# bdsaglam/torch-scae

Hardware: AMD Instinct MI355X
Metric: images/sec SCAE fwd+bwd, MNIST 40x40 bs=128, 1/2/4/8 MI355X (higher is better)
Workload: dtype f32

## Files before the change

### torch_scae_amd/csrc/seed_attention_wave.hip

```cpp
#include <algorithm>

#include "wave_mfma.h"

using namespace scae_wave;

namespace {
constexpr int NTH = 256;

struct SwArgs {
  const float *h;
  const float *q;
  const float *wk;
  const float *wv, *bv;
  const float *presence;
  float *out;
  const float *gout;
  float *gh;
  float *partial;
  int B, N, O, C;
  float inv_sqrt_c;
  int bf16;
};

enum { T_QK = 0, T_TS, T_DT, T_QKT, T_TT, T_DTT, T_SMALL };
// ... 162 lines not shown
  fold_qk<NT>(a, l, tl, false);
  for (int b = blockIdx.x; b < a.B; b += gridDim.x) {
    if (l.v < NT && 16 * l.v < O) {
      const int t = l.v;
      const Keys<NT> k = load_keys<NT>(a, b, l);
      f32x4 p[NT];
      probabilities<NT, BF>(a, l, tl, t, k, p);
      wr_nn<NT>(tl.large(T_PS), t, l, p);
      lds_fence();
      const f32x4 T = mmakp<NT, BF>(splat(0.f), rdk<NT>(tl.large(T_PS), t, l), k.hT);
      wr_rows(tl.small(T_TS), t, l, T);
      lds_fence();
    }
    __syncthreads();
    float *ob = a.out + (size_t)b * O * C;
    for (int ct = l.v; ct * 16 < C; ct += 4) {
      const float4 wb = ld4(a.wv + (size_t)(16 * ct + l.r) * D + 4 * l.q);
      const float bias = a.bv[16 * ct + l.r];
#pragma unroll
      for (int t = 0; t < NT; ++t) {
        if (16 * t >= O) break;
        const f32x4 o = mma16(splat(bias), rd16(tl.small(T_TS), t, l), wb);
#pragma unroll
        for (int e = 0; e < 4; ++e) {
          const int row = 16 * t + 4 * l.q + e;
          if (row < O) ob[(size_t)row * C + 16 * ct + l.r] = o[e];
        }
      }
    }
    __syncthreads();
  }
}

template <int NT, bool BF>
__device__ __forceinline__ f32x4 saw_bwd_body(const SwArgs &a, float *smem, int blk, int nblk) {
  const Tl<NT> tl{smem};
  const Lane l = make_lane();
  const int C = a.C, O = a.O, N = a.N, CW = C / 4, run = CW / 4;
  constexpr int TSN = Geo<NT>::TSN;
  const int npar = O * D + C * D + C;
  float *part = a.partial + (size_t)blk * npar;
  float *scr = tl.scr();
  static_assert(Geo<NT>::LDS_FLOATS % 4 == 0, "16-byte zero fill");
  for (int i = 4 * threadIdx.x; i < Geo<NT>::LDS_FLOATS; i += 4 * NTH)
    *reinterpret_cast<float4 *>(smem + i) = make_float4(0.f, 0.f, 0.f, 0.f);
  __syncthreads();
  fold_qk<NT>(a, l, tl, true);
  bool first = true;
  auto put = [&](int idx, float v) { part[idx] = first ? v : part[idx] + v; };
  const int k0 = CW * l.v + run * l.q;
  f32x4 gh_tile = splat(0.f);
  for (int b = blk; b < a.B; b += nblk) {
    const float *gb = a.gout + (size_t)b * O * C;
    {
      f32x4 acc[NT];
#pragma unroll
      for (int t = 0; t < NT; ++t) acc[t] = splat(0.f);
      for (int j = 0; j < run; j += 4) {
        const float *wp = a.wv + (size_t)(k0 + j) * D + l.r;
        const float4 wb = make_float4(wp[0], wp[D], wp[2 * D], wp[3 * D]);
#pragma unroll
        for (int t = 0; t < NT; ++t) {
          const int o = 16 * t + l.r;
          const float4 av =
              o < O ? ld4(gb + (size_t)o * C + k0 + j) : make_float4(0.f, 0.f, 0.f, 0.f);
          acc[t] = mma16(acc[t], av, wb);
        }
      }
#pragma unroll
      for (int t = 0; t < NT; ++t)
#pragma unroll
        for (int e = 0; e < 4; ++e)
          scr[((l.v * NT + t) * 16 + 4 * l.q + e) * D + l.r] = acc[t][e];
    }
    Keys<NT> k;
    f32x4 p[NT];
    const bool qwave = l.v < NT && 16 * l.v < O;
    if (qwave) {
      const int t = l.v;
      k = load_keys<NT>(a, b, l);
      probabilities<NT, BF>(a, l, tl, t, k, p);
      wr_nn<NT>(tl.large(T_PS), t, l, p);
      wr_nn_t<NT>(tl.large(T_PT), t, l, p);
      lds_fence();
      const f32x4 T = mmakp<NT, BF>(splat(0.f), rdk<NT>(tl.large(T_PS), t, l), k.hT);
      wr_cols<NT>(tl.small(T_TT), t, l, T);
    }
    lds_fence();
    __syncthreads();
    for (int i = threadIdx.x; i < Geo<NT>::ROWS * D; i += NTH) {
      const float s =
          (scr[i] + scr[NT * 256 + i]) + (scr[2 * NT * 256 + i] + scr[3 * NT * 256 + i]);
      const int o = i / D, c = i % D;
      tl.small(T_DT)[o * RS + c] = s;
      tl.small(T_DTT)[c * TSN + o] = s;
    }
    __syncthreads();
    {
      const FK<NT> tb = rdk<NT>(tl.small(T_TT), 0, l);
      for (int ct = l.v; ct * 16 < C; ct += 4) {
        FK<NT> ga;
        float cs = 0.f;
#pragma unroll
        for (int j = 0; j < NT; ++j) {
          float g[4];
#pragma unroll
          for (int s = 0; s < 4; ++s) {
            const int o = 4 * NT * l.q + 4 * j + s;
            g[s] = o < O ? gb[(size_t)o * C + 16 * ct + l.r] : 0.f;
          }
          ga.v[j] = make_float4(g[0], g[1], g[2], g[3]);
          cs += (g[0] + g[1]) + (g[2] + g[3]);
        }
        const f32x4 dw = mmak<NT>(splat(0.f), ga, tb);
#pragma unroll
        for (int e = 0; e < 4; ++e) put(O * D + (16 * ct + 4 * l.q + e) * D + l.r, dw[e]);
        cs += __shfl_xor(cs, 16, 64);
        cs += __shfl_xor(cs, 32, 64);
        if (l.q == 0) put(O * D + C * D + 16 * ct + l.r, cs);
      }
    }
    if (qwave) {
      const int t = l.v;
      const float4 dta = rd16(tl.small(T_DT), t, l);
      f32x4 ds[NT];
#pragma unroll
      for (int u = 0; u < NT; ++u) ds[u] = mma16p<BF>(splat(0.f), dta, k.hB[u]);
#pragma unroll
      for (int e = 0; e < 4; ++e) {
        float dot = 0.f;
#pragma unroll
        for (int u = 0; u < NT; ++u) dot = fmaf(p[u][e], ds[u][e], dot);
        dot = rsum(dot);
#pragma unroll
        for (int u = 0; u < NT; ++u) ds[u][e] = p[u][e] * (ds[u][e] - dot) * a.inv_sqrt_c;
      }
      wr_nn<NT>(tl.large(T_DSR), t, l, ds);
      wr_nn_t<NT>(tl.large(T_DST), t, l, ds);
      lds_fence();
      const f32x4 dqk = mmakp<NT, BF>(splat(0.f), rdk<NT>(tl.large(T_DSR), t, l), k.hT);
#pragma unroll
      for (int e = 0; e < 4; ++e) {
        const int o = 16 * t + 4 * l.q + e;
        if (o < O) put(o * D + l.r, dqk[e]);
      }
    }
    lds_fence();
    __syncthreads();
    if (l.v < NT && 16 * l.v < N) {
      const int u = l.v;
      f32x4 gh = mmakp<NT, BF>(splat(0.f), rdk<NT>(tl.large(T_PT), u, l), rdk<NT>(tl.small(T_DTT), 0, l));
      gh = mmakp<NT, BF>(gh, rdk<NT>(tl.large(T_DST), u, l), rdk<NT>(tl.small(T_QKT), 0, l));
#pragma unroll
      for (int e = 0; e < 4; ++e) {
        const int n = 16 * u + 4 * l.q + e;
        if (n < N) a.gh[((size_t)b * N + n) * D + l.r] = gh[e];
      }
      gh_tile = gh;
    }
    first = false;
    __syncthreads();
  }
  return gh_tile;
}
template <int NT, bool BF>
__global__ __launch_bounds__(NTH) void saw_bwd_kernel(SwArgs a) {
  extern __shared__ __attribute__((aligned(16))) float smem[];
  saw_bwd_body<NT, BF>(a, smem, blockIdx.x, gridDim.x);
}

constexpr int RTH = 1024;
struct ReduceArgs {
  const float *partial;
  int rows;
  const float *q, *wk;
  float *gq, *gwk, *gbk, *gwv, *gbv;
  int O, C, nsum;
};
inline int reduce_blocks(const ReduceArgs &r, int RT) {
  return r.nsum + (r.O * r.C + r.C * D + RT - 1) / RT;
}
template <int RT>
__device__ __forceinline__ void saw_reduce_body(const ReduceArgs &a, float *lds, int blk) {
  constexpr int VR = RTH / RT;
  float (*red)[65] = reinterpret_cast<float (*)[65]>(lds);
  float *dqk = lds + 16 * 65;
  const float *__restrict__ partial = a.partial;
  const int rows = a.rows, O = a.O, C = a.C, nsum = a.nsum;
  const int npar = O * D + C * D + C;
  const int cx = threadIdx.x & 63, ry0 = (threadIdx.x >> 6) * VR;
  auto colsum = [&](int col, bool ok) {
#pragma unroll
    for (int vr = 0; vr < VR; ++vr) {
      const int ry = ry0 + vr;
      float acc = 0.f;
      if (ok) {
// ... 143 lines not shown
```

### torch_scae_amd/csrc/seed_bwd_gemm.hip

```cpp
#include <algorithm>

#include "mfma_tile.h"
#include "set_encoder_args.h"
#include "wave_mfma.h"

#define SCAE_DEVICE_ONLY
namespace scae_saw {
#include "seed_attention_wave.hip"
}
namespace scae_gemm {
#include "gemm_mfma.hip"
}
#include "set_encoder_wave.hip"
#undef SCAE_DEVICE_ONLY

namespace {
constexpr int NTH = 256;
static_assert(scae_tile::NT == NTH, "one block size for both parts");

template <int NT, bool BF>
__global__ __launch_bounds__(NTH) void saw_bwd_gemm_kernel(scae_saw::SwArgs a, int n_saw,
                                                           scae_gemm::GemmMulti p) {
  extern __shared__ __attribute__((aligned(16))) float smem[];
  if ((int)blockIdx.x < n_saw)
    scae_saw::saw_bwd_body<NT, BF>(a, smem, blockIdx.x, n_saw);
  else
    scae_gemm::gemm_multi_body<1>(p, smem, (int)blockIdx.x - n_saw);
}

template <int NT, bool BF>
int launch(const scae_saw::SwArgs &a, const scae_gemm::GemmMulti &p, hipStream_t st) {
  const size_t lds = sizeof(float) * std::max<size_t>(scae_saw::Geo<NT>::LDS_FLOATS,
                                                      scae_tile::Tile<1>::SMEM);
// ... 31 lines not shown
__global__ __launch_bounds__(NTH) __attribute__((amdgpu_waves_per_eu(2)))
void saw_stw_bwd_gemm_kernel(scae_saw::SwArgs a, int n_saw,
                                                               scae_gemm::GemmMulti p,
                                                               scae_st::StArgs t,
                                                               int trunk_lds_floats) {
  extern __shared__ __attribute__((aligned(16))) float smem[];
  if ((int)blockIdx.x >= n_saw) {
    scae_gemm::gemm_multi_body<1>(p, smem, (int)blockIdx.x - n_saw);
    return;
  }
  const scae_wave::f32x4 gh = scae_saw::saw_bwd_body<2, BF>(a, smem, blockIdx.x, n_saw);
  scae_st::lds_zero(smem, trunk_lds_floats, threadIdx.x, NTH);
  scae_wave::lds_fence();
  __syncthreads();
  if (threadIdx.x >= 64 * NTS) return;
  scae_st::stw_bwd_body<NTS, BF, true>(t, smem, blockIdx.x, n_saw, gh);
}

template <int NTS, bool BF>
int launch_trunk(const scae_saw::SwArgs &a, const scae_gemm::GemmMulti &p,
                 const scae_st::StArgs &t, hipStream_t st) {
  const size_t trunk = scae_st::stw_bwd_lds_floats<NTS>(t.Din);
  const size_t lds =
      sizeof(float) * std::max<size_t>({scae_saw::Geo<2>::LDS_FLOATS, scae_tile::Tile<1>::SMEM, trunk});
  if (lds > 48 * 1024) {
    hipError_t e = hipFuncSetAttribute(
        reinterpret_cast<const void *>(saw_stw_bwd_gemm_kernel<NTS, BF>),
        hipFuncAttributeMaxDynamicSharedMemorySize, (int)lds);
    if (e != hipSuccess) return (int)e;
  }
  scae::launch((saw_stw_bwd_gemm_kernel<NTS, BF>), dim3(a.B + p.first[p.n]), dim3(NTH), lds, st,
               a, a.B, p, t, (int)trunk);
  return scae_launch_status();
}

bool trunk_rides(int B, int N, int O, int C, int D, int Din, int Dout, int L, int layer_norm) {
  return B > 0 && B <= 512 && N > 0 && N <= 32 && O > 0 && O <= 32 && C > 0 && (C & 63) == 0 &&
         D == scae_wave::D && Dout == 0 && scae_st::wave_bwd_shape(N, D, Din, Dout, L, layer_norm);
}

int impl_trunk(const float *h, const float *q, const float *wk, const float *wv,
               const float *presence, const float *gout, float *gh, float *partial, int B, int N,
               int O, int C, const scae_gemm_desc *descs, int n, int nseg,
               const float *const *seg_ptr, const int *seg_width, const int *seg_row_stride,
               const int64_t *seg_batch_stride, float *const *seg_grad,
               const float *trunk_presence, const float *params, const float *hsave,
               float *pg_partial, int B2, int N2, int D, int Din, int Dout, int L, int layer_norm,
               int bf16, void *stream) {
  SCAE_REQUIRE(h && q && wk && wv && gout && gh && partial && descs);
  if (B2 != B || N2 != N) return SCAE_ERR_BAD_ARG;
  scae_saw::SwArgs a{h,  q,       wk, wv, nullptr, presence, nullptr, gout,
                     gh, partial, B,  N,  O,       C,        1.f / sqrtf((float)C), bf16};
  int rc = scae_saw::check(a);
  if (rc) return rc;
  scae_st::StArgs t;
  rc = scae_st::wave_bwd_args(t, bf16 != 0, nseg, seg_ptr, seg_width, seg_row_stride,
                              seg_batch_stride, seg_grad, trunk_presence, params, hsave,
                              pg_partial, B, N, D, Din, Dout, L, layer_norm);
  if (rc) return rc;
  scae_gemm::GemmMulti p;
  int T;
  rc = scae_gemm::plan_multi(p, T, descs, n);
  if (rc) return rc;
  if (T != 32) return SCAE_ERR_UNSUPPORTED;
  if (!trunk_rides(B, N, O, C, D, Din, Dout, L, layer_norm)) return SCAE_ERR_UNSUPPORTED;
  hipStream_t st = (hipStream_t)stream;
  if (N <= 16) return bf16 ? launch_trunk<1, true>(a, p, t, st) : launch_trunk<1, false>(a, p, t, st);
  return bf16 ? launch_trunk<2, true>(a, p, t, st) : launch_trunk<2, false>(a, p, t, st);
}
}

extern "C" int scae_object_encoder_bwd_supported(int B, int N, int O, int C, int D, int Din,
                                                 int Dout, int L, int layer_norm) {
  return trunk_rides(B, N, O, C, D, Din, Dout, L, layer_norm) ? 1 : 0;
}
#define SCAE_OBJECT_ENCODER_BWD(SUFFIX, BF)                                                      \
  extern "C" int scae_object_encoder_bwd_gemm_##SUFFIX(                                          \
      const float *h, const float *q, const float *wk, const float *wv, const float *presence,   \
      const float *gout, float *gh, float *partial, int B, int N, int O, int C,                  \
      const scae_gemm_desc *descs, int n, int nseg, const float *const *seg_ptr,                 \
      const int *seg_width, const int *seg_row_stride, const int64_t *seg_batch_stride,          \
      float *const *seg_grad, const float *trunk_presence, const float *params,                  \
      const float *hsave, float *pg_partial, int trunk_B, int trunk_N, int D, int Din, int Dout, \
      int L, int layer_norm, void *stream) {                                                     \
    return impl_trunk(h, q, wk, wv, presence, gout, gh, partial, B, N, O, C, descs, n, nseg,     \
                      seg_ptr, seg_width, seg_row_stride, seg_batch_stride, seg_grad,            \
                      trunk_presence, params, hsave, pg_partial, trunk_B, trunk_N, D, Din, Dout, \
                      L, layer_norm, BF, stream);                                                \
  }
SCAE_OBJECT_ENCODER_BWD(f32, 0)
SCAE_OBJECT_ENCODER_BWD(bf16, 1)
#undef SCAE_OBJECT_ENCODER_BWD

extern "C" int scae_seed_attention_mfma_bwd_gemm_f32(
    const float *h, const float *q, const float *wk, const float *wv, const float *presence,
    const float *gout, float *gh, float *partial, int B, int N, int O, int C,
    const scae_gemm_desc *descs, int n, void *stream) {
  return impl(h, q, wk, wv, presence, gout, gh, partial, B, N, O, C, descs, n, 0, stream);
}
extern "C" int scae_seed_attention_mfma_bwd_gemm_bf16(
    const float *h, const float *q, const float *wk, const float *wv, const float *presence,
    const float *gout, float *gh, float *partial, int B, int N, int O, int C,
    const scae_gemm_desc *descs, int n, void *stream) {
// ... 3 lines not shown
```

### torch_scae_amd/csrc/set_encoder_wave.hip

```cpp
#include "set_encoder_args.h"
#include "wave_mfma.h"

#pragma clang fp contract(off)

namespace scae_st {
namespace {
using namespace scae_wave;

#ifdef SCAE_STW_PROF
__device__ unsigned long long g_stw_prof[160];
__device__ int g_stw_n;
#define STW_T()                                                                  \
  do {                                                                           \
    if (blockIdx.x == 5 && threadIdx.x == 0) {                                   \
      const int i_ = g_stw_n;                                                    \
      if (i_ < 160) g_stw_prof[i_] = __builtin_readcyclecounter(), g_stw_n = i_ + 1; \
    }                                                                            \
  } while (0)
#else
#define STW_T()
#endif

struct Lay {
  int Din, L, ln;
  __device__ int b1() const { return D * Din; }
  __device__ int layer(int l) const { return D * Din + D + l * (5 * 272 + (ln ? 64 : 0)); }
  __device__ int w(int m) const { return m < 4 ? m * 272 : 4 * 272 + (ln ? 32 : 0); }
  __device__ int b(int m) const { return w(m) + 256; }
  __device__ int ln0() const { return 4 * 272; }
  __device__ int ln1() const { return b(4) + 16; }
  __device__ int total() const { return layer(L); }
};

struct Wave {
  int lane, r, q, t;
  int ts;
  __device__ __forceinline__ void wr_rows(float *tile, const f32x4 &o) const {
#pragma unroll
    for (int e = 0; e < 4; ++e) tile[(16 * t + 4 * q + e) * RS + r] = o[e];
  }
  __device__ __forceinline__ void wr_cols(float *tile, const f32x4 &o) const {
    *reinterpret_cast<float4 *>(tile + r * ts + 16 * t + 4 * q) =
        make_float4(o[0], o[1], o[2], o[3]);
  }
  template <int NT>
  __device__ __forceinline__ void wr_nn(float *tile, const f32x4 (&o)[NT]) const {
#pragma unroll
    for (int u = 0; u < NT; ++u)
#pragma unroll
      for (int e = 0; e < 4; ++e) tile[(16 * t + 4 * q + e) * ts + 16 * u + r] = o[u][e];
  }
  template <int NT>
  __device__ __forceinline__ void wr_nn_t(float *tile, const f32x4 (&o)[NT]) const {
#pragma unroll
    for (int u = 0; u < NT; ++u)
      *reinterpret_cast<float4 *>(tile + (16 * u + r) * ts + 16 * t + 4 * q) =
          make_float4(o[u][0], o[u][1], o[u][2], o[u][3]);
  }
  __device__ __forceinline__ float4 rd16(const float *tile, int u) const {
    return ld4(tile + (16 * u + r) * RS + 4 * q);
  }
  template <int NT>
  __device__ __forceinline__ FK<NT> rdk(const float *tile, int u) const {
    const float *p = tile + (16 * u + r) * ts + 4 * NT * q;
    FK<NT> f;
#pragma unroll
    for (int j = 0; j < NT; ++j) f.v[j] = ld4(p + 4 * j);
    return f;
// ... 42 lines not shown
  f32x4 h1;
  f32x4 tv;
  f32x4 xh0, rstd0, xh1, rstd1;
};

template <int NT>
struct Geo {
  static constexpr int TSN = 16 * NT + 8;
  static constexpr int SMALL = 16 * NT * RS > 16 * TSN ? 16 * NT * RS : 16 * TSN;
  static constexpr int LARGE = 16 * NT * TSN;
  static constexpr int SCR = NT * (5 * 256 + 10 * D);
};
enum {
  S_HS = 0, S_QS,
  S_KS0, S_VT0,
  S_BWD_FIRST,
  S_KS1 = S_BWD_FIRST, S_VT1, S_FWD_SMALL,
  S_VS = S_BWD_FIRST, S_KT, S_QT, S_GT,
  S_XT1, S_XT2,
  S_BWD_SMALL
};
constexpr int S_AS = S_HS, S_GR = S_HS, S_H1S = S_QS;
enum { L_PS = 0, L_FWD_LARGE, L_PT = L_FWD_LARGE, L_DST, L_BWD_LARGE };
constexpr int L_DSR = L_PS;
template <int NT>
struct Tiles {
  float *base;
  float *lbase;
  float *scr;
  __device__ __forceinline__ float *small(int i) const { return base + i * Geo<NT>::SMALL; }
  __device__ __forceinline__ float *large(int i) const { return lbase + i * Geo<NT>::LARGE; }
};

template <int NT, bool KEEP, bool BF>
__device__ __forceinline__ void sab_forward(const Wave &w, const Lay &lay, const float *Wl,
                                            const Tiles<NT> &tl, f32x4 &h, const f32x4 &pres,
                                            const float (&kmask)[NT], int N, float sqrt_d,
                                            int par, SabState<NT> *st) {
  float *Hs = tl.small(S_HS), *Qs = tl.small(S_QS), *As = tl.small(S_AS),
        *H1s = tl.small(S_H1S), *Ps = tl.large(L_PS),
        *Ks = tl.small(!KEEP && par ? S_KS1 : S_KS0),
        *Vt = tl.small(!KEEP && par ? S_VT1 : S_VT0);
  const int r = w.r, t = w.t;
  const float inv_sqrt_d = 1.f / sqrt_d;
  const float4 wq = w.w_rows(Wl + lay.w(0)), wk = w.w_rows(Wl + lay.w(1)),
               wv = w.w_rows(Wl + lay.w(2)), wo = w.w_rows(Wl + lay.w(3)),
               wf = w.w_rows(Wl + lay.w(4));
  const float bq = Wl[lay.b(0) + r], bk = Wl[lay.b(1) + r], bv = Wl[lay.b(2) + r],
              bo = Wl[lay.b(3) + r], bf = Wl[lay.b(4) + r];
  float g0 = 1.f, be0 = 0.f, g1 = 1.f, be1 = 0.f;
  if (lay.ln) {
    g0 = Wl[lay.ln0() + r], be0 = Wl[lay.ln0() + D + r];
    g1 = Wl[lay.ln1() + r], be1 = Wl[lay.ln1() + D + r];
  }
  if (KEEP) st->hin = h;
  STW_T();
  w.wr_rows(Hs, h);
  lds_fence();
  f32x4 qo, ko, vo;
  {
    const float4 a = w.rd16(Hs, t);
    qo = mma16(splat(bq), a, wq);
    ko = mma16(splat(bk), a, wk);
    vo = mma16(splat(bv), a, wv);
  }
  w.wr_rows(Qs, qo);
  w.wr_rows(Ks, ko);
  w.wr_cols(Vt, vo);
  if (KEEP) {
    w.wr_rows(tl.small(S_VS), vo);
    w.wr_cols(tl.small(S_KT), ko);
    w.wr_cols(tl.small(S_QT), qo);
  }
  lds_fence();
  if (NT > 1) __syncthreads();
  STW_T();
  f32x4 s[NT];
  {
    const float4 qa = w.rd16(Qs, t);
#pragma unroll
    for (int u = 0; u < NT; ++u) s[u] = mma16p<BF>(splat(0.f), qa, w.rd16(Ks, u));
  }
  STW_T();
#pragma unroll
  for (int e = 0; e < 4; ++e) {
    float v[NT], mx = -INFINITY, sum = 0.f;
#pragma unroll
    for (int u = 0; u < NT; ++u) {
      v[u] = 16 * u + r < N ? (s[u][e] - kmask[u]) * inv_sqrt_d : -INFINITY;
      mx = fmaxf(mx, v[u]);
    }
    mx = rmax(mx);
#pragma unroll
    for (int u = 0; u < NT; ++u) v[u] = __expf(v[u] - mx), sum += v[u];
#ifdef SCAE_NO_RCP
    const float inv = 1.f / rsum(sum);
#else
    const float inv = __builtin_amdgcn_rcpf(rsum(sum));
#endif
#pragma unroll
    for (int u = 0; u < NT; ++u) s[u][e] = v[u] * inv;
  }
  if (KEEP) {
#pragma unroll
    for (int u = 0; u < NT; ++u) st->p[u] = s[u];
  }
  STW_T();
  w.template wr_nn<NT>(Ps, s);
  lds_fence();
  const f32x4 ao = mma_np<NT, BF>(splat(0.f), w, Ps, t, Vt, 0);
  if (KEEP) st->ao = ao;
  STW_T();
  w.wr_rows(As, ao);
  lds_fence();
  f32x4 h1 = mma16(splat(bo), w.rd16(As, t), wo);
#pragma unroll
  for (int e = 0; e < 4; ++e) h1[e] = (h1[e] + h[e]) * pres[e];
  f32x4 dummy;
  if (lay.ln) layer_norm<KEEP>(h1, g0, be0, KEEP ? st->xh0 : dummy, KEEP ? st->rstd0 : dummy);
  STW_T();
  w.wr_rows(H1s, h1);
  lds_fence();
  const f32x4 tv = mma16(splat(bf), w.rd16(H1s, t), wf);
  if (KEEP) st->tv = tv, st->h1 = h1;
#pragma unroll
  for (int e = 0; e < 4; ++e) h[e] = h1[e] + fmaxf(tv[e], 0.f);
  if (lay.ln) layer_norm<KEEP>(h, g1, be1, KEEP ? st->xh1 : dummy, KEEP ? st->rstd1 : dummy);
  STW_T();
}

__host__ __device__ inline int xs_of(int Din) { return (Din + 15) / 16 * 16 + 4; }
template <int NT>
__host__ __device__ inline size_t lds_floats_fwd_aliased(int Din) {
  const size_t xw = (size_t)(16 * NT + 16) * xs_of(Din),
               tl = (size_t)S_FWD_SMALL * Geo<NT>::SMALL + (size_t)L_FWD_LARGE * Geo<NT>::LARGE;
  return xw > tl ? xw : tl;
}
template <int NT>
__host__ __device__ inline size_t lds_floats(int Din, bool bwd) {
  const size_t xs = xs_of(Din);
  if (!bwd)
    return (16 * NT + 16) * xs + (size_t)S_FWD_SMALL * Geo<NT>::SMALL +
           (size_t)L_FWD_LARGE * Geo<NT>::LARGE;
  return (size_t)S_BWD_SMALL * Geo<NT>::SMALL + Geo<NT>::SCR +
         (size_t)L_BWD_LARGE * Geo<NT>::LARGE;
}

typedef __amdgpu_buffer_rsrc_t rsrc_t;
__device__ __forceinline__ rsrc_t make_rsrc(const void *p) {
  return __builtin_amdgcn_make_buffer_rsrc(const_cast<void *>(p), 0, 0x7ffffffc, 0x00020000);
}
__device__ __forceinline__ void dma4(rsrc_t r, float *lds, int voff, int soff) {
  __builtin_amdgcn_raw_ptr_buffer_load_lds(r, (__attribute__((address_space(3))) void *)lds, 4,
                                           voff, soff, 0, 0);
}
__device__ __forceinline__ void dma_rows(const float *src, int sstride, int n0, int n1, int width,
                                         float *dst, int XS, int lane, int nstep = 1) {
  const rsrc_t rs = make_rsrc(src);
  for (int c = 0; c < width; c += 64)
    if (c + lane < width)
      for (int n = n0; n < n1; n += nstep)
        dma4(rs, dst + n * XS + c, 4 * lane, 4 * (n * sstride + c));
// ... 71 lines not shown
    h0 = mma16(h0, ld4(xa + j), ld4(wb + j));
    h1 = mma16(h1, ld4(xa + j + 4), ld4(wb + j + 4));
  }
  if (j < kq) h0 = mma16(h0, ld4(xa + j), ld4(wb + j));
  return h0 + h1;
}

__device__ __forceinline__ float4 rdT_own(const Wave &w, const float *tile) {
  return ld4(tile + w.r * w.ts + 16 * w.t + 4 * w.q);
}
__device__ __forceinline__ void layer_norm_bwd(f32x4 &g, float gamma, const f32x4 &xh,
                                               const f32x4 &rstd, float &dgamma, float &dbeta) {
  f32x4 gx;
#pragma unroll
  for (int e = 0; e < 4; ++e) gx[e] = g[e] * xh[e];
  dgamma = csum(gx);
  dbeta = csum(g);
#pragma unroll
  for (int e = 0; e < 4; ++e) {
    const float gh = g[e] * gamma;
    const float s1 = rsum(gh) * (1.f / D), s2 = rsum(gh * xh[e]) * (1.f / D);
    g[e] = (gh - s1 - xh[e] * s2) * rstd[e];
  }
}
struct LayerGrads {
  f32x4 w[5];
  float v[9];
};

template <int NT, bool BF>
__device__ __forceinline__ void sab_backward(const Wave &w, const Lay &lay, const float *Wl,
                                             const Tiles<NT> &tl, f32x4 &G, const f32x4 &pres,
                                             int N, float sqrt_d, const SabState<NT> &st,
                                             LayerGrads &lg) {
  float *XT1 = tl.small(S_XT1), *XT2 = tl.small(S_XT2), *GR = tl.small(S_GR),
        *GT = tl.small(S_GT), *Vs = tl.small(S_VS), *Kt = tl.small(S_KT),
        *Qt = tl.small(S_QT), *PT = tl.large(L_PT), *DSR = tl.large(L_DSR),
        *DST = tl.large(L_DST);
  const int r = w.r, t = w.t;
  const float inv_sqrt_d = 1.f / sqrt_d;
  const float4 wqT = w.w_cols(Wl + lay.w(0)), wkT = w.w_cols(Wl + lay.w(1)),
               wvT = w.w_cols(Wl + lay.w(2)), woT = w.w_cols(Wl + lay.w(3)),
               wfT = w.w_cols(Wl + lay.w(4));
#pragma unroll
  for (int i = 5; i < 9; ++i) lg.v[i] = 0.f;
  if (lay.ln) layer_norm_bwd(G, Wl[lay.ln1() + r], st.xh1, st.rstd1, lg.v[7], lg.v[8]);
  f32x4 gt;
#pragma unroll
  for (int e = 0; e < 4; ++e) gt[e] = st.tv[e] > 0.f ? G[e] : 0.f;
  w.wr_cols(XT1, gt);
  w.wr_cols(XT2, st.h1);
  w.wr_rows(GR, gt);
  lds_fence();
  lg.w[4] = mma16(splat(0.f), rdT_own(w, XT1), rdT_own(w, XT2));
  lg.v[4] = csum(gt);
  f32x4 g1 = mma16(G, w.rd16(GR, t), wfT);
  STW_T();
  if (lay.ln) layer_norm_bwd(g1, Wl[lay.ln0() + r], st.xh0, st.rstd0, lg.v[5], lg.v[6]);
  f32x4 go;
#pragma unroll
  for (int e = 0; e < 4; ++e) go[e] = g1[e] * pres[e];
  w.wr_cols(XT1, go);
  w.wr_cols(XT2, st.ao);
  w.wr_rows(GR, go);
  lds_fence();
  lg.w[3] = mma16(splat(0.f), rdT_own(w, XT1), rdT_own(w, XT2));
  lg.v[3] = csum(go);
  const f32x4 ga = mma16(splat(0.f), w.rd16(GR, t), woT);
  STW_T();
  w.wr_rows(GR, ga);
  w.wr_cols(GT, ga);
// ... 46 lines not shown
                                            const LayerGrads &lg, float *part, bool first) {
  constexpr int PW = 5 * 256 + 10 * D;
  auto put = [&](int idx, float v) { part[idx] = first ? v : part[idx] + v; };
  if (NT == 1) {
#pragma unroll
    for (int m = 0; m < 5; ++m)
#pragma unroll
      for (int e = 0; e < 4; ++e) put(lay.w(m) + (4 * w.q + e) * D + w.r, lg.w[m][e]);
    if (w.q == 0) {
      const int voff[9] = {lay.b(0), lay.b(1), lay.b(2), lay.b(3), lay.b(4), lay.ln0(),
                           lay.ln0() + D, lay.ln1(), lay.ln1() + D};
#pragma unroll
      for (int i = 0; i < 9; ++i)
        if (i < 5 || lay.ln) put(voff[i] + w.r, lg.v[i]);
    }
    return;
  }
  float *mine = tl.scr + w.t * PW;
#pragma unroll
  for (int m = 0; m < 5; ++m)
#pragma unroll
    for (int e = 0; e < 4; ++e) mine[m * 256 + (4 * w.q + e) * D + w.r] = lg.w[m][e];
  if (w.q == 0) {
#pragma unroll
    for (int i = 0; i < 9; ++i) mine[5 * 256 + i * D + w.r] = lg.v[i];
  }
  lds_fence();
  __syncthreads();
  static_assert(D == 16, "vector index split");
  constexpr int NTH = 64 * NT, NI = 5 * 64 + 9 * 4, ITS = (NI + NTH - 1) / NTH;
  float4 v[ITS];
#pragma unroll
  for (int it = 0; it < ITS; ++it) {
    const int k = 4 * min((int)threadIdx.x + NTH * it, NI - 1);
    float4 o = make_float4(0.f, 0.f, 0.f, 0.f);
#pragma unroll
    for (int t = 1; t < NT; ++t) {
      const float4 x = ld4(tl.scr + t * PW + k);
      o.x += x.x, o.y += x.y, o.z += x.z, o.w += x.w;
    }
    const float4 x = ld4(tl.scr + k);
    v[it] = make_float4(x.x + o.x, x.y + o.y, x.z + o.z, x.w + o.w);
  }
#pragma unroll
  for (int it = 0; it < ITS; ++it) {
    const int item = (int)threadIdx.x + NTH * it, k = 4 * item;
    const int m = k >> 8, iv = (k - 5 * 256) >> 4;
    const int wm = m * 272 + (m == 4 && lay.ln ? 32 : 0);
    const int vo = iv < 5 ? iv * 272 + (iv == 4 && lay.ln ? 32 : 0) + 256
                          : iv == 5 ? lay.ln0()
                                    : iv == 6 ? lay.ln0() + D : iv == 7 ? lay.ln1() : lay.ln1() + D;
    const bool mat = k < 5 * 256;
    if (item < NI && (mat || iv < 5 || lay.ln)) {
      float4 *dst = reinterpret_cast<float4 *>(part + (mat ? wm + (k & 255) : vo + (k & 15)));
      float4 r = v[it];
      if (!first) {
        const float4 p = *dst;
        r.x += p.x, r.y += p.y, r.z += p.z, r.w += p.w;
      }
      *dst = r;
    }
  }
}

template <int NT, bool BF, bool HANDED>
__device__ __forceinline__ void stw_bwd_body(const StArgs &a, float *smem, int blk, int nblk,
                                             f32x4 G_in) {
  const Lay lay{a.Din, a.L, a.layer_norm};
  const int N = a.N, Din = a.Din;
  Wave w;
  w.lane = threadIdx.x & 63, w.r = w.lane & 15, w.q = w.lane >> 4;
  w.t = __builtin_amdgcn_readfirstlane(threadIdx.x >> 6);
  w.ts = Geo<NT>::TSN;
  float *sm = smem, *scr = sm + S_BWD_SMALL * Geo<NT>::SMALL, *arena = scr + Geo<NT>::SCR;
  const Tiles<NT> tiles{sm, arena, scr};
  const int lds_total = (int)lds_floats<NT>(Din, true);
#ifdef SCAE_STW_PROF
  if (blockIdx.x == 5 && threadIdx.x == 0) g_stw_n = 0;
#endif
  STW_T();
  if (!HANDED) {
    lds_zero(smem, lds_total, threadIdx.x, 64 * NT);
    lds_fence();
    if (NT > 1) __syncthreads();
  }
  float *part = a.pg_partial + (size_t)blk * lay.total();
  STW_T();
  bool first = true;
  for (int b = blk; b < a.B; b += nblk) {
    f32x4 pres, G;
    float kmask[NT];
#pragma unroll
    for (int e = 0; e < 4; ++e) {
      const int n = 16 * w.t + 4 * w.q + e;
      pres[e] = n < N ? (a.presence ? a.presence[(size_t)b * N + n] : 1.f) : 0.f;
      G[e] = n < N ? (HANDED ? G_in[e] : a.gz[((size_t)b * N + n) * D + w.r]) : 0.f;
    }
#pragma unroll
    for (int u = 0; u < NT; ++u) {
      const int m = 16 * u + w.r;
      kmask[u] = a.presence && m < N ? (1.f - a.presence[(size_t)b * N + m]) * 1e32f : 0.f;
    }
    const float *hs = a.hsave + (size_t)b * (a.L + 1) * N * D;
    for (int l = a.L - 1; l >= 0; --l) {
      f32x4 h;
#pragma unroll
      for (int e = 0; e < 4; ++e) {
        const int n = 16 * w.t + 4 * w.q + e;
        h[e] = n < N ? hs[((size_t)l * N + n) * D + w.r] : 0.f;
      }
      SabState<NT> st;
      const float *Wl = a.params + lay.layer(l);
      sab_forward<NT, true, BF>(w, lay, Wl, tiles, h, pres, kmask, N, a.sqrt_d, 0, &st);
      LayerGrads lg;
      sab_backward<NT, BF>(w, lay, Wl, tiles, G, pres, N, a.sqrt_d, st, lg);
      flush_layer<NT>(w, lay, tiles, lg, part + lay.layer(l), first);
  STW_T();
    }
    float *GT = tiles.small(S_GT), *GR = tiles.small(S_GR);
    constexpr int XT = NT <= 2 ? 5 : (NT == 3 ? 3 : 2);
    constexpr int WT = 10;
    const int ntile = (Din + 15) / 16;
    struct Col {
      const float *x;
      float *g;
      int rs, wd;
    };
    auto column = [&](int c) {
      Col k{nullptr, nullptr, 0, 0};
      int c0 = 0;
#pragma unroll
      for (int sgi = 0; sgi < MAXSEG; ++sgi) {
        if (sgi < a.nseg) {
          const Seg &sg = a.seg[sgi];
          if (c >= c0) {
            k.x = sg.ptr + (size_t)b * sg.bs + (c - c0);
            k.g = sg.grad ? sg.grad + (size_t)b * N * sg.width + (c - c0) : nullptr;
// ... 93 lines not shown
#pragma unroll
              for (int e = 0; e < 4; ++e) {
                const int n = 16 * w.t + 4 * w.q + e;
                if (n < N) k.g[(size_t)n * k.wd] = gx[i][e];
              }
            }
          }
        }
        jx += NT * XT, jw += WT;
        if (jx < ntile) load_x(jx);
        if (jw < ntile) load_w(jw);
      } while (jx < ntile || jw < ntile);
    }
    first = false;
  STW_T();
    if (HANDED) break;
    if (NT > 1) __syncthreads();
  }
}

template <int NT, bool BF>
__global__ __launch_bounds__(64 * NT) void stw_bwd_kernel(StArgs a) {
  extern __shared__ __attribute__((aligned(16))) float smem[];
  stw_bwd_body<NT, BF, false>(a, smem, blockIdx.x, gridDim.x, splat(0.f));
}

template <int NT, bool BF, bool ALIAS = false>
__device__ __forceinline__ void stw_fwd_body(const StArgs &a, float *smem, int blk_id, int nblk) {
  const Lay lay{a.Din, a.L, a.layer_norm};
  const int N = a.N, XS = xs_of(a.Din);
  Wave w;
  w.lane = threadIdx.x & 63, w.r = w.lane & 15, w.q = w.lane >> 4;
  w.t = __builtin_amdgcn_readfirstlane(threadIdx.x >> 6);
  w.ts = Geo<NT>::TSN;
  float *X = smem, *W1s = X + 16 * NT * XS, *sm = ALIAS ? smem : W1s + 16 * XS;
  const Tiles<NT> tiles{sm, sm + S_FWD_SMALL * Geo<NT>::SMALL, nullptr};
  lds_zero(X, (16 * NT + 16) * XS, threadIdx.x, 64 * NT);
  lds_fence();
  if (NT > 1) __syncthreads();
  NarrowRows nr;
  if (blk_id < a.B) stage_input_issue(a, blk_id, w, X, XS, nr);
  dma_rows(a.params, a.Din, w.t, D, a.Din, W1s, XS, w.lane, NT);
  int blk = 0;
  for (int b = blk_id; b < a.B; b += nblk) {
    if (b != blk_id) {
      if (ALIAS) {
        if (NT > 1) __syncthreads();
        lds_zero(X, (16 * NT + 16) * XS, threadIdx.x, 64 * NT);
        lds_fence();
        if (NT > 1) __syncthreads();
        dma_rows(a.params, a.Din, w.t, D, a.Din, W1s, XS, w.lane, NT);
      }
      stage_input_issue(a, b, w, X, XS, nr);
    }
    f32x4 pres;
    float kmask[NT];
#pragma unroll
    for (int e = 0; e < 4; ++e) {
      const int n = 16 * w.t + 4 * w.q + e;
      pres[e] = n < N ? (a.presence ? a.presence[(size_t)b * N + n] : 1.f) : 0.f;
    }
#pragma unroll
    for (int u = 0; u < NT; ++u) {
      const int m = 16 * u + w.r;
      kmask[u] = a.presence && m < N ? (1.f - a.presence[(size_t)b * N + m]) * 1e32f : 0.f;
    }
// ... 106 lines not shown
```

Before: 272,300.

## Overlap trunk top-layer forward recompute with idle waves of seed-attention backward

Adds an early fused kernel in which the waves left idle during the seed-attention backward phases (probabilities, softmax backward, dh) recompute the set-encoder trunk's last-layer forward. That recompute is split into stages slotted into those idle points, and its Q/K/V tiles and saved state are kept in LDS for the trunk backward. This removes one layer of serial forward recomputation from the trunk backward's critical path. The kernel is enabled by default through an environment variable, limits LDS so two workgroups fit per CU, and remaps the trunk to start at wave 2, which raises register pressure and code complexity.

```diff
diff --git a/torch_scae_amd/csrc/seed_attention_wave.hip b/torch_scae_amd/csrc/seed_attention_wave.hip
--- a/torch_scae_amd/csrc/seed_attention_wave.hip
+++ b/torch_scae_amd/csrc/seed_attention_wave.hip
@@ -218,8 +218,15 @@
   }
 }
 
-template <int NT, bool BF>
-__device__ __forceinline__ f32x4 saw_bwd_body(const SwArgs &a, float *smem, int blk, int nblk) {
+struct NoIdleWork {
+  __device__ __forceinline__ void at_set_start() const {}
+  __device__ __forceinline__ void in_probabilities() const {}
+  __device__ __forceinline__ void in_softmax_bwd() const {}
+  __device__ __forceinline__ void in_dh() const {}
+};
+template <int NT, bool BF, bool ONE_SET = false, class Idle>
+__device__ __forceinline__ f32x4 saw_bwd_body(const SwArgs &a, float *smem, int blk, int nblk,
+                                              Idle &idle) {
   const Tl<NT> tl{smem};
   const Lane l = make_lane();
   const int C = a.C, O = a.O, N = a.N, CW = C / 4, run = CW / 4;
@@ -238,6 +245,7 @@
   f32x4 gh_tile = splat(0.f);
   for (int b = blk; b < a.B; b += nblk) {
     const float *gb = a.gout + (size_t)b * O * C;
+    idle.at_set_start();
     {
       f32x4 acc[NT];
 #pragma unroll
@@ -271,6 +279,8 @@
       lds_fence();
       const f32x4 T = mmakp<NT, BF>(splat(0.f), rdk<NT>(tl.large(T_PS), t, l), k.hT);
       wr_cols<NT>(tl.small(T_TT), t, l, T);
+    } else {
+      idle.in_probabilities();
     }
     lds_fence();
     __syncthreads();
@@ -330,6 +340,8 @@
         const int o = 16 * t + 4 * l.q + e;
         if (o < O) put(o * D + l.r, dqk[e]);
       }
+    } else {
+      idle.in_softmax_bwd();
     }
     lds_fence();
     __syncthreads();
@@ -343,11 +355,19 @@
         if (n < N) a.gh[((size_t)b * N + n) * D + l.r] = gh[e];
       }
       gh_tile = gh;
+    } else {
+      idle.in_dh();
     }
     first = false;
     __syncthreads();
+    if (ONE_SET) break;
   }
   return gh_tile;
+}
+template <int NT, bool BF>
+__device__ __forceinline__ f32x4 saw_bwd_body(const SwArgs &a, float *smem, int blk, int nblk) {
+  NoIdleWork idle;
+  return saw_bwd_body<NT, BF, false>(a, smem, blk, nblk, idle);
 }
 template <int NT, bool BF>
 __global__ __launch_bounds__(NTH) void saw_bwd_kernel(SwArgs a) {
diff --git a/torch_scae_amd/csrc/seed_bwd_gemm.hip b/torch_scae_amd/csrc/seed_bwd_gemm.hip
--- a/torch_scae_amd/csrc/seed_bwd_gemm.hip
+++ b/torch_scae_amd/csrc/seed_bwd_gemm.hip
@@ -1,4 +1,5 @@
 #include <algorithm>
+#include <cstdlib>
 
 #include "mfma_tile.h"
 #include "set_encoder_args.h"
@@ -96,6 +97,75 @@
   scae::launch((saw_stw_bwd_gemm_kernel<NTS, BF>), dim3(a.B + p.first[p.n]), dim3(NTH), lds, st,
                a, a.B, p, t, (int)trunk);
   return scae_launch_status();
+}
+
+constexpr int EARLY_WAVE0 = 2;
+template <int NTS, bool BF>
+struct EarlyTrunk {
+  scae_st::EarlyBlock<NTS, BF> blk;
+  const scae_st::StArgs &t;
+  __device__ __forceinline__ explicit EarlyTrunk(const scae_st::StArgs &t_) : t(t_) {}
+  __device__ __forceinline__ void at_set_start() { blk.load(t); }
+  __device__ __forceinline__ void in_probabilities() { blk.probabilities(); }
+  __device__ __forceinline__ void in_softmax_bwd() { blk.pv_oproj(); }
+  __device__ __forceinline__ void in_dh() { blk.ff(); }
+};
+template <int NTS>
+size_t early_keep_off(size_t trunk) {
+  return std::max<size_t>(scae_saw::Geo<2>::LDS_FLOATS + scae_st::EarlyGeo<NTS>::WORK, trunk);
+}
+template <int NTS, bool BF>
+__global__ __launch_bounds__(NTH) __attribute__((amdgpu_waves_per_eu(2)))
+void saw_stw_bwd_gemm_early_kernel(scae_saw::SwArgs a, int n_saw, scae_gemm::GemmMulti p,
+                                   scae_st::StArgs t, int trunk_lds_floats, int keep_off) {
+  extern __shared__ __attribute__((aligned(16))) float smem[];
+  if ((int)blockIdx.x >= n_saw) {
+    scae_gemm::gemm_multi_body<1>(p, smem, (int)blockIdx.x - n_saw);
+    return;
+  }
+  const int wave = __builtin_amdgcn_readfirstlane(threadIdx.x >> 6);
+  float *keep = smem + keep_off, *hand = keep + scae_st::EarlyGeo<NTS>::KEEP;
+  EarlyTrunk<NTS, BF> idle(t);
+  idle.blk.init(t, blockIdx.x, wave, EARLY_WAVE0, smem + scae_saw::Geo<2>::LDS_FLOATS, keep);
+  const scae_wave::f32x4 gh = scae_saw::saw_bwd_body<2, BF, true>(a, smem, blockIdx.x, n_saw, idle);
+  if (wave < NTS)
+    *reinterpret_cast<float4 *>(hand + 4 * threadIdx.x) = make_float4(gh[0], gh[1], gh[2], gh[3]);
+  scae_st::lds_zero(smem, trunk_lds_floats, threadIdx.x, NTH);
+  scae_wave::lds_fence();
+  __syncthreads();
+  if (wave < EARLY_WAVE0 || wave >= EARLY_WAVE0 + NTS) return;
+  const float4 g = *reinterpret_cast<const float4 *>(hand + 4 * (threadIdx.x - 64 * EARLY_WAVE0));
+  scae_wave::f32x4 G;
+  G[0] = g.x, G[1] = g.y, G[2] = g.z, G[3] = g.w;
+  scae_st::stw_bwd_body<NTS, BF, true, true>(t, smem, blockIdx.x, n_saw, G, &idle.blk.st, keep,
+                                             EARLY_WAVE0);
+}
+
+template <int NTS, bool BF>
+int launch_trunk_early(const scae_saw::SwArgs &a, const scae_gemm::GemmMulti &p,
+                       const scae_st::StArgs &t, hipStream_t st) {
+  const size_t trunk = scae_st::stw_bwd_lds_floats<NTS>(t.Din), keep = early_keep_off<NTS>(trunk);
+  const size_t lds = sizeof(float) * std::max<size_t>(
+      scae_tile::Tile<1>::SMEM, keep + scae_st::EarlyGeo<NTS>::KEEP + scae_st::EarlyGeo<NTS>::HAND);
+  static_assert(sizeof(float) * (scae_saw::Geo<2>::LDS_FLOATS + scae_st::EarlyGeo<NTS>::WORK +
+                                 scae_st::EarlyGeo<NTS>::KEEP + scae_st::EarlyGeo<NTS>::HAND) <=
+                    80 * 1024, "two workgroups per CU");
+  if (lds > 80 * 1024) return SCAE_ERR_UNSUPPORTED;
+  hipError_t e = hipFuncSetAttribute(
+      reinterpret_cast<const void *>(saw_stw_bwd_gemm_early_kernel<NTS, BF>),
+      hipFuncAttributeMaxDynamicSharedMemorySize, (int)lds);
+  if (e != hipSuccess) return (int)e;
+  scae::launch((saw_stw_bwd_gemm_early_kernel<NTS, BF>), dim3(a.B + p.first[p.n]), dim3(NTH), lds,
+               st, a, a.B, p, t, (int)trunk, (int)keep);
+  return scae_launch_status();
+}
+
+bool trunk_overlap() {
+  static const bool on = [] {
+    const char *e = std::getenv("SCAE_TRUNK_OVERLAP");
+    return !(e && e[0] == '0' && !e[1]);
+  }();
+  return on;
 }
 
 bool trunk_rides(int B, int N, int O, int C, int D, int Din, int Dout, int L, int layer_norm) {
@@ -129,10 +199,26 @@
   if (T != 32) return SCAE_ERR_UNSUPPORTED;
   if (!trunk_rides(B, N, O, C, D, Din, Dout, L, layer_norm)) return SCAE_ERR_UNSUPPORTED;
   hipStream_t st = (hipStream_t)stream;
+  if (trunk_overlap()) {
+    if (N <= 16)
+      return bf16 ? launch_trunk_early<1, true>(a, p, t, st) : launch_trunk_early<1, false>(a, p, t, st);
+    return bf16 ? launch_trunk_early<2, true>(a, p, t, st) : launch_trunk_early<2, false>(a, p, t, st);
+  }
   if (N <= 16) return bf16 ? launch_trunk<1, true>(a, p, t, st) : launch_trunk<1, false>(a, p, t, st);
   return bf16 ? launch_trunk<2, true>(a, p, t, st) : launch_trunk<2, false>(a, p, t, st);
 }
 }
+
+#ifdef SCAE_STW_PROF
+extern "C" int scae_debug_oe_prof(unsigned long long *out, int n) {
+  int cnt = 0;
+  (void)hipDeviceSynchronize();
+  if (hipMemcpyFromSymbol(&cnt, HIP_SYMBOL(scae_st::g_stw_n), sizeof(int)) != hipSuccess) return -1;
+  if (cnt > n) cnt = n;
+  if (hipMemcpyFromSymbol(out, HIP_SYMBOL(scae_st::g_stw_prof), cnt * 8) != hipSuccess) return -1;
+  return cnt;
+}
+#endif
 
 extern "C" int scae_object_encoder_bwd_supported(int B, int N, int O, int C, int D, int Din,
                                                  int Dout, int L, int layer_norm) {
diff --git a/torch_scae_amd/csrc/set_encoder_wave.hip b/torch_scae_amd/csrc/set_encoder_wave.hip
--- a/torch_scae_amd/csrc/set_encoder_wave.hip
+++ b/torch_scae_amd/csrc/set_encoder_wave.hip
@@ -12,7 +12,7 @@
 __device__ int g_stw_n;
 #define STW_T()                                                                  \
   do {                                                                           \
-    if (blockIdx.x == 5 && threadIdx.x == 0) {                                   \
+    if (blockIdx.x == 5 && w.tid == 0) {                                         \
       const int i_ = g_stw_n;                                                    \
       if (i_ < 160) g_stw_prof[i_] = __builtin_readcyclecounter(), g_stw_n = i_ + 1; \
     }                                                                            \
@@ -34,6 +34,7 @@
 
 struct Wave {
   int lane, r, q, t;
+  int tid;
   int ts;
   __device__ __forceinline__ void wr_rows(float *tile, const f32x4 &o) const {
 #pragma unroll
@@ -142,6 +143,78 @@
   __device__ __forceinline__ float *large(int i) const { return lbase + i * Geo<NT>::LARGE; }
 };
 
+template <int NT, bool BF>
+__device__ __forceinline__ void sab_probs(const Wave &w, const float *Qs, const float *Ks,
+                                          const float (&kmask)[NT], int N, float inv_sqrt_d,
+                                          f32x4 (&s)[NT]) {
+  const int r = w.r, t = w.t;
+  {
+    const float4 qa = w.rd16(Qs, t);
+#pragma unroll
+    for (int u = 0; u < NT; ++u) s[u] = mma16p<BF>(splat(0.f), qa, w.rd16(Ks, u));
+  }
+  STW_T();
+#pragma unroll
+  for (int e = 0; e < 4; ++e) {
+    float v[NT], mx = -INFINITY, sum = 0.f;
+#pragma unroll
+    for (int u = 0; u < NT; ++u) {
+      v[u] = 16 * u + r < N ? (s[u][e] - kmask[u]) * inv_sqrt_d : -INFINITY;
+      mx = fmaxf(mx, v[u]);
+    }
+    mx = rmax(mx);
+#pragma unroll
+    for (int u = 0; u < NT; ++u) v[u] = __expf(v[u] - mx), sum += v[u];
+#ifdef SCAE_NO_RCP
+    const float inv = 1.f / rsum(sum);
+#else
+    const float inv = __builtin_amdgcn_rcpf(rsum(sum));
+#endif
+#pragma unroll
+    for (int u = 0; u < NT; ++u) s[u][e] = v[u] * inv;
+  }
+  STW_T();
+}
+template <int NT, bool BF>
+__device__ __forceinline__ f32x4 sab_pv(const Wave &w, float *Ps, const float *Vt,
+                                        const f32x4 (&s)[NT]) {
+  w.template wr_nn<NT>(Ps, s);
+  lds_fence();
+  const f32x4 ao = mma_np<NT, BF>(splat(0.f), w, Ps, w.t, Vt, 0);
+  STW_T();
+  return ao;
+}
+template <int NT, bool KEEP>
+__device__ __forceinline__ f32x4 sab_oproj(const Wave &w, int ln, float *As, const f32x4 &ao,
+                                           const f32x4 &h, const f32x4 &pres, const float4 &wo,
+                                           float bo, float g0, float be0, SabState<NT> *st) {
+  w.wr_rows(As, ao);
+  lds_fence();
+  f32x4 h1 = mma16(splat(bo), w.rd16(As, w.t), wo);
+#pragma unroll
+  for (int e = 0; e < 4; ++e) h1[e] = (h1[e] + h[e]) * pres[e];
+  f32x4 dummy;
+  if (ln) layer_norm<KEEP>(h1, g0, be0, KEEP ? st->xh0 : dummy, KEEP ? st->rstd0 : dummy);
+  STW_T();
+  return h1;
+}
+template <int NT, bool KEEP>
+__device__ __forceinline__ f32x4 sab_ff(const Wave &w, int ln, float *H1s, const f32x4 &h1,
+                                        const float4 &wf, float bf, float g1, float be1,
+                                        SabState<NT> *st) {
+  w.wr_rows(H1s, h1);
+  lds_fence();
+  const f32x4 tv = mma16(splat(bf), w.rd16(H1s, w.t), wf);
+  if (KEEP) st->tv = tv, st->h1 = h1;
+  f32x4 h;
+#pragma unroll
+  for (int e = 0; e < 4; ++e) h[e] = h1[e] + fmaxf(tv[e], 0.f);
+  f32x4 dummy;
+  if (ln) layer_norm<KEEP>(h, g1, be1, KEEP ? st->xh1 : dummy, KEEP ? st->rstd1 : dummy);
+  STW_T();
+  return h;
+}
+
 template <int NT, bool KEEP, bool BF>
 __device__ __forceinline__ void sab_forward(const Wave &w, const Lay &lay, const float *Wl,
                                             const Tiles<NT> &tl, f32x4 &h, const f32x4 &pres,
@@ -186,58 +259,129 @@
   if (NT > 1) __syncthreads();
   STW_T();
   f32x4 s[NT];
-  {
-    const float4 qa = w.rd16(Qs, t);
-#pragma unroll
-    for (int u = 0; u < NT; ++u) s[u] = mma16p<BF>(splat(0.f), qa, w.rd16(Ks, u));
-  }
-  STW_T();
-#pragma unroll
-  for (int e = 0; e < 4; ++e) {
-    float v[NT], mx = -INFINITY, sum = 0.f;
+  sab_probs<NT, BF>(w, Qs, Ks, kmask, N, inv_sqrt_d, s);
+  const f32x4 ao = sab_pv<NT, BF>(w, Ps, Vt, s);
+  if (KEEP) {
+#pragma unroll
+    for (int u = 0; u < NT; ++u) st->p[u] = s[u];
+    st->ao = ao;
+  }
+  const f32x4 h1 = sab_oproj<NT, KEEP>(w, lay.ln, As, ao, h, pres, wo, bo, g0, be0, st);
+  h = sab_ff<NT, KEEP>(w, lay.ln, H1s, h1, wf, bf, g1, be1, st);
+}
+
+template <int NT>
+struct EarlyGeo {
+  static constexpr int TSN = Geo<NT>::TSN;
+  static constexpr int WAVE = 16 * RS + 16 * NT * RS + 2 * 16 * TSN;
+  static constexpr int WORK = NT * WAVE;
+  static constexpr int KEEP = 3 * Geo<NT>::SMALL;
+  static constexpr int HAND = NT * 256;
+};
+template <int NT, bool BF>
+struct EarlyBlock {
+  Wave w;
+  bool on;
+  int ln, N;
+  float inv_sqrt_d;
+  const float *Wl, *hs;
+  float *rt, *ks, *vt, *ps, *keep;
+  const float *prow;
+  float4 wq, wk, wv, wo, wf, ha[NT];
+  f32x4 bias;
+  f32x4 ffv;
+  f32x4 ln0v;
+  float kmask[NT];
+  f32x4 pres;
+  SabState<NT> st;
+  f32x4 h1;
+
+  __device__ __forceinline__ void init(const StArgs &a, int b, int wave, int wave0, float *work,
+                                       float *keep_) {
+    w.lane = threadIdx.x & 63, w.r = w.lane & 15, w.q = w.lane >> 4;
+    w.t = wave - wave0;
+    w.tid = (int)threadIdx.x - 64 * wave0;
+    w.ts = Geo<NT>::TSN;
+    on = wave >= wave0 && wave < wave0 + NT && a.L > 0;
+    ln = a.layer_norm, N = a.N, inv_sqrt_d = 1.f / a.sqrt_d;
+    const Lay lay{a.Din, a.L, a.layer_norm};
+    Wl = a.params + lay.layer(a.L - 1);
+    hs = a.hsave + ((size_t)b * (a.L + 1) + (a.L - 1)) * a.N * D;
+    float *mine = work + w.t * EarlyGeo<NT>::WAVE;
+    rt = mine - 16 * w.t * RS;
+    ks = mine + 16 * RS;
+    vt = ks + 16 * NT * RS;
+    ps = vt + 16 * w.ts - 16 * w.t * w.ts;
+    keep = keep_;
+    prow = a.presence ? a.presence + (size_t)b * N : nullptr;
+  }
+  __device__ __forceinline__ void load(const StArgs &a) {
+    if (!on) return;
+#ifdef SCAE_STW_PROF
+    if (blockIdx.x == 5 && w.tid == 0) g_stw_n = 0;
+#endif
+    STW_T();
+    const Lay lay{a.Din, a.L, ln};
+    const int r = w.r, q = w.q;
+    wq = w.w_rows(Wl + lay.w(0)), wk = w.w_rows(Wl + lay.w(1)), wv = w.w_rows(Wl + lay.w(2));
+    wo = w.w_rows(Wl + lay.w(3)), wf = w.w_rows(Wl + lay.w(4));
+    bias[0] = Wl[lay.b(0) + r], bias[1] = Wl[lay.b(1) + r], bias[2] = Wl[lay.b(2) + r];
+    bias[3] = Wl[lay.b(3) + r], ffv[0] = Wl[lay.b(4) + r];
+    ffv[3] = Wl[ln ? lay.ln0() + r : r], ln0v = splat(Wl[ln ? lay.ln0() + D + r : r]);
+    ffv[1] = Wl[ln ? lay.ln1() + r : r], ffv[2] = Wl[ln ? lay.ln1() + D + r : r];
 #pragma unroll
     for (int u = 0; u < NT; ++u) {
-      v[u] = 16 * u + r < N ? (s[u][e] - kmask[u]) * inv_sqrt_d : -INFINITY;
-      mx = fmaxf(mx, v[u]);
-    }
-    mx = rmax(mx);
-#pragma unroll
-    for (int u = 0; u < NT; ++u) v[u] = __expf(v[u] - mx), sum += v[u];
-#ifdef SCAE_NO_RCP
-    const float inv = 1.f / rsum(sum);
-#else
-    const float inv = __builtin_amdgcn_rcpf(rsum(sum));
-#endif
-#pragma unroll
-    for (int u = 0; u < NT; ++u) s[u][e] = v[u] * inv;
-  }
-  if (KEEP) {
-#pragma unroll
-    for (int u = 0; u < NT; ++u) st->p[u] = s[u];
-  }
-  STW_T();
-  w.template wr_nn<NT>(Ps, s);
-  lds_fence();
-  const f32x4 ao = mma_np<NT, BF>(splat(0.f), w, Ps, t, Vt, 0);
-  if (KEEP) st->ao = ao;
-  STW_T();
-  w.wr_rows(As, ao);
-  lds_fence();
-  f32x4 h1 = mma16(splat(bo), w.rd16(As, t), wo);
-#pragma unroll
-  for (int e = 0; e < 4; ++e) h1[e] = (h1[e] + h[e]) * pres[e];
-  f32x4 dummy;
-  if (lay.ln) layer_norm<KEEP>(h1, g0, be0, KEEP ? st->xh0 : dummy, KEEP ? st->rstd0 : dummy);
-  STW_T();
-  w.wr_rows(H1s, h1);
-  lds_fence();
-  const f32x4 tv = mma16(splat(bf), w.rd16(H1s, t), wf);
-  if (KEEP) st->tv = tv, st->h1 = h1;
-#pragma unroll
-  for (int e = 0; e < 4; ++e) h[e] = h1[e] + fmaxf(tv[e], 0.f);
-  if (lay.ln) layer_norm<KEEP>(h, g1, be1, KEEP ? st->xh1 : dummy, KEEP ? st->rstd1 : dummy);
-  STW_T();
-}
+      const int m = 16 * u + r, mc = min(m, N - 1);
+      const float pm = prow ? prow[mc] : 1.f;
+      const float4 hv = ld4(hs + (size_t)mc * D + 4 * q);
+      kmask[u] = prow && m < N ? (1.f - pm) * 1e32f : 0.f;
+      ha[u] = m < N ? hv : make_float4(0.f, 0.f, 0.f, 0.f);
+    }
+#pragma unroll
+    for (int e = 0; e < 4; ++e) {
+      const int n = 16 * w.t + 4 * q + e, nc = min(n, N - 1);
+      const float hv = hs[(size_t)nc * D + r], pn = prow ? prow[nc] : 1.f;
+      st.hin[e] = n < N ? hv : 0.f;
+      pres[e] = n < N ? pn : 0.f;
+    }
+    STW_T();
+  }
+  __device__ __forceinline__ void probabilities() {
+    if (!on) return;
+    STW_T();
+    const int r = w.r, q = w.q;
+    float *Vs = keep, *Kt = keep + Geo<NT>::SMALL, *Qt = keep + 2 * Geo<NT>::SMALL;
+#pragma unroll
+    for (int u = 0; u < NT; ++u) {
+      const f32x4 ko = mma16(splat(bias[1]), ha[u], wk), vo = mma16(splat(bias[2]), ha[u], wv);
+#pragma unroll
+      for (int e = 0; e < 4; ++e) ks[(16 * u + 4 * q + e) * RS + r] = ko[e];
+      *reinterpret_cast<float4 *>(vt + r * w.ts + 16 * u + 4 * q) =
+          make_float4(vo[0], vo[1], vo[2], vo[3]);
+      if (u == w.t) {
+        const f32x4 qo = mma16(splat(bias[0]), ha[u], wq);
+        w.wr_rows(rt, qo);
+        w.wr_rows(Vs, vo);
+        w.wr_cols(Kt, ko);
+        w.wr_cols(Qt, qo);
+      }
+    }
+    lds_fence();
+    STW_T();
+    sab_probs<NT, BF>(w, rt, ks, kmask, N, inv_sqrt_d, st.p);
+  }
+  __device__ __forceinline__ void pv_oproj() {
+    if (!on) return;
+    STW_T();
+    st.ao = sab_pv<NT, BF>(w, ps, vt, st.p);
+    h1 = sab_oproj<NT, true>(w, ln, rt, st.ao, st.hin, pres, wo, bias[3], ffv[3], ln0v[0], &st);
+  }
+  __device__ __forceinline__ void ff() {
+    if (!on) return;
+    STW_T();
+    sab_ff<NT, true>(w, ln, rt, h1, wf, ffv[0], ffv[1], ffv[2], &st);
+  }
+};
 
 __host__ __device__ inline int xs_of(int Din) { return (Din + 15) / 16 * 16 + 4; }
 template <int NT>
@@ -375,11 +519,13 @@
 __device__ __forceinline__ void sab_backward(const Wave &w, const Lay &lay, const float *Wl,
                                              const Tiles<NT> &tl, f32x4 &G, const f32x4 &pres,
                                              int N, float sqrt_d, const SabState<NT> &st,
-                                             LayerGrads &lg) {
+                                             LayerGrads &lg, const float *keep = nullptr) {
   float *XT1 = tl.small(S_XT1), *XT2 = tl.small(S_XT2), *GR = tl.small(S_GR),
-        *GT = tl.small(S_GT), *Vs = tl.small(S_VS), *Kt = tl.small(S_KT),
-        *Qt = tl.small(S_QT), *PT = tl.large(L_PT), *DSR = tl.large(L_DSR),
+        *GT = tl.small(S_GT), *PT = tl.large(L_PT), *DSR = tl.large(L_DSR),
         *DST = tl.large(L_DST);
+  const float *Vs = keep ? keep : tl.small(S_VS),
+              *Kt = keep ? keep + Geo<NT>::SMALL : tl.small(S_KT),
+              *Qt = keep ? keep + 2 * Geo<NT>::SMALL : tl.small(S_QT);
   const int r = w.r, t = w.t;
   const float inv_sqrt_d = 1.f / sqrt_d;
   const float4 wqT = w.w_cols(Wl + lay.w(0)), wkT = w.w_cols(Wl + lay.w(1)),
@@ -492,7 +638,7 @@
   float4 v[ITS];
 #pragma unroll
   for (int it = 0; it < ITS; ++it) {
-    const int k = 4 * min((int)threadIdx.x + NTH * it, NI - 1);
+    const int k = 4 * min(w.tid + NTH * it, NI - 1);
     float4 o = make_float4(0.f, 0.f, 0.f, 0.f);
 #pragma unroll
     for (int t = 1; t < NT; ++t) {
@@ -504,7 +650,7 @@
   }
 #pragma unroll
   for (int it = 0; it < ITS; ++it) {
-    const int item = (int)threadIdx.x + NTH * it, k = 4 * item;
+    const int item = w.tid + NTH * it, k = 4 * item;
     const int m = k >> 8, iv = (k - 5 * 256) >> 4;
     const int wm = m * 272 + (m == 4 && lay.ln ? 32 : 0);
     const int vo = iv < 5 ? iv * 272 + (iv == 4 && lay.ln ? 32 : 0) + 256
@@ -523,24 +669,27 @@
   }
 }
 
-template <int NT, bool BF, bool HANDED>
+template <int NT, bool BF, bool HANDED, bool EARLY = false>
 __device__ __forceinline__ void stw_bwd_body(const StArgs &a, float *smem, int blk, int nblk,
-                                             f32x4 G_in) {
+                                             f32x4 G_in, const SabState<NT> *early = nullptr,
+                                             const float *keep = nullptr, int wave0 = 0) {
+  static_assert(HANDED || !EARLY, "an early block belongs to the handed form");
   const Lay lay{a.Din, a.L, a.layer_norm};
   const int N = a.N, Din = a.Din;
   Wave w;
   w.lane = threadIdx.x & 63, w.r = w.lane & 15, w.q = w.lane >> 4;
-  w.t = __builtin_amdgcn_readfirstlane(threadIdx.x >> 6);
+  w.t = __builtin_amdgcn_readfirstlane((int)(threadIdx.x >> 6) - wave0);
+  w.tid = (int)threadIdx.x - 64 * wave0;
   w.ts = Geo<NT>::TSN;
   float *sm = smem, *scr = sm + S_BWD_SMALL * Geo<NT>::SMALL, *arena = scr + Geo<NT>::SCR;
   const Tiles<NT> tiles{sm, arena, scr};
   const int lds_total = (int)lds_floats<NT>(Din, true);
 #ifdef SCAE_STW_PROF
-  if (blockIdx.x == 5 && threadIdx.x == 0) g_stw_n = 0;
+  if (blockIdx.x == 5 && w.tid == 0 && !(EARLY && a.L > 0)) g_stw_n = 0;
 #endif
   STW_T();
   if (!HANDED) {
-    lds_zero(smem, lds_total, threadIdx.x, 64 * NT);
+    lds_zero(smem, lds_total, w.tid, 64 * NT);
     lds_fence();
     if (NT > 1) __syncthreads();
   }
@@ -562,7 +711,16 @@
       kmask[u] = a.presence && m < N ? (1.f - a.presence[(size_t)b * N + m]) * 1e32f : 0.f;
     }
     const float *hs = a.hsave + (size_t)b * (a.L + 1) * N * D;
-    for (int l = a.L - 1; l >= 0; --l) {
+    int l = a.L - 1;
+    if (EARLY && l >= 0) {
+      const float *Wl = a.params + lay.layer(l);
+      LayerGrads lg;
+      sab_backward<NT, BF>(w, lay, Wl, tiles, G, pres, N, a.sqrt_d, *early, lg, keep);
+      flush_layer<NT>(w, lay, tiles, lg, part + lay.layer(l), first);
+  STW_T();
+      --l;
+    }
+    for (; l >= 0; --l) {
       f32x4 h;
 #pragma unroll
       for (int e = 0; e < 4; ++e) {
@@ -722,6 +880,7 @@
   Wave w;
   w.lane = threadIdx.x & 63, w.r = w.lane & 15, w.q = w.lane >> 4;
   w.t = __builtin_amdgcn_readfirstlane(threadIdx.x >> 6);
+  w.tid = threadIdx.x;
   w.ts = Geo<NT>::TSN;
   float *X = smem, *W1s = X + 16 * NT * XS, *sm = ALIAS ? smem : W1s + 16 * XS;
   const Tiles<NT> tiles{sm, sm + S_FWD_SMALL * Geo<NT>::SMALL, nullptr};
```

After: 273,300 (median of 3 runs). About the same (+0.4%).
